# codybloemhard/termdaw

Measured on AMD Instinct MI355X. Metric: offline render Msamples/sec (stereo 48 kHz) + % HBM roofline, 64-vertex graph, higher is better.
Workload: dtype f32; 1 GPU; BASELINE config 2: 64 sampleloop -> 1 normalize, 60 s @48 kHz, bl 1024, 16-bit PCM out; 1 project(s) per GPU per step (project p of the job on rank p mod N, seed offset 64*p); frames_per_project=2880512, projects_per_gpu=1, vertices_per_project=65, normalize=one launch, output=int16 PCM in HBM, parallelism=project p on rank p mod N; one RCCL all-reduce(max) of the 1-entry peak table

## Files before the change

termdaw_amd/csrc/compile.cpp:

```cpp
#include "chorus_math.h"
#include "compile.h"
#include "delay_math.h"
#include "eq_math.h"
#include "sat_math.h"

#include <math.h>
#include <stdlib.h>
#include <string.h>

#include <algorithm>
#include <chrono>
#include <limits>

using namespace tdk;

namespace tde {

const char* const kFamilyName[F_COUNT] = {"k_sample_loop", "k_sample_multi", "k_sample_lerp", "k_debug_sine",
                                           "k_synth",       "k_sampsyn", "k_adsr_env", "k_sine_probe", "k_sum",          "k_scale",       "k_norm_fix",
                                           "k_adsr",        "k_band_pass",    "k_band_spec", "k_band_fix", "k_band_fill", "k_band_scan", "k_quantise", "k_band_audit", "k_stems", "k_sources", "k_loudness",
                                           "k_master_detect", "k_master_scan", "k_master_carry", "k_master_apply",
                                           "k_comp_detect", "k_comp_carry_y1", "k_comp_env", "k_comp_carry_yl", "k_comp_apply",
                                           "k_eq_local", "k_eq_carry", "k_eq_apply",
                                           "k_delay_local", "k_delay_carry", "k_delay_apply",
// ... 1366 lines not shown
            if (!adsr_through.empty()) term_mode[vi] = ins.size() == 1 ? TERMS_ADSR1 : TERMS_WITH_ADSR;
            for (const auto& th : adsr_through) {
                const size_t a = th.second;
                const Vertex& av = g->vertices[a];
                AdsrVDesc x{};
                x.tab.n_int = vt[a].n_int;
                x.k = 1u;
                x.sr = (uint32_t)sr;
                x.bl = (uint32_t)bl;
                x.use_off = av.use_off;
                x.use_max = av.use_max;
                x.wet = av.wet;
                x.conf = av.conf;
                x.pg = make_pg(av.gain, av.angle);
                adsr_fill_run_consts(&x);
                x.env = env_of[a];
                const size_t in_off = st.put(std::vector<InTerm>{plain_term(g->edges[a][0])});
                const size_t o = st.alloc(sizeof x);
                memcpy(&st.b[o], &x, sizeof x);
                ptr_field(o, offsetof(AdsrVDesc, ins), in_off);
                const size_t t = o + offsetof(AdsrVDesc, tab);
                tab_field(t, offsetof(IntervalTab, istart), vt[a], vt[a].istart_off);
                tab_field(t, offsetof(IntervalTab, tile_first), vt[a], vt[a].tile_first_off);
                tab_field(t, offsetof(IntervalTab, ivoff), vt[a], vt[a].ivoff_off);
                tab_field(t, offsetof(IntervalTab, voices), vt[a], vt[a].voices_off);
                ptr_field(ins_off[vi] + th.first * sizeof(InTerm), offsetof(InTerm, len), o);
            }
        }
        for (size_t vi : norm_pending) {
            const Vertex& v = g->vertices[vi];
            uint32_t mode = 1u;
            if (g->spec_normalize && !is_scan) {
                const uint32_t tm = term_mode[vi];
                const bool wide = (tm == TERMS_ALL_LOOP16 || tm == TERMS_ALL_LOOP32) && bl == (size_t)kTileFrames &&
                                  M >= (size_t)1800 * kTileFrames && M < ((size_t)1 << 31);
                if (v.peak_known && !v.has_init_override) mode = 3u;
                else if (!wide && g->single_pass_normalize && bl == (size_t)kTileFrames && M < ((size_t)1 << 31)) {
                    const int tpw = norm1_tiles_per_workgroup(tm, (uint32_t)M);
                    if (tpw) { mode = 5u; norm_tpw[vi] = tpw; }
                } else if (wide && g->single_pass_normalize) {
                    const bool packed = tm == TERMS_ALL_LOOP16;
                    const int nq = (packed && M >= (size_t)2600 * kTileFrames) ? 4 : 2;
                    const size_t gx = (M + (size_t)kTileFrames * nq - 1) / ((size_t)kTileFrames * nq);
                    mode = (size_t)sum16w_resident_capacity(nq, packed) >= gx ? 5u : 4u;
                }
            }
            norm_mode[vi] = mode;
            fam_v[mode == 1u ? F_SCALE : F_NORMFIX].push_back(vi);
        }
        std::map<size_t, std::pair<size_t, size_t>> norm_scratch;
        std::map<size_t, SumDesc> sum_desc_of;
        size_t band_desc_off = 0;
        uint32_t max_nseg = 0;
        for (int fam = 0; fam < F_COUNT; ++fam) {
            auto& vs = fam_v[fam];
            if (fam == F_BAND_FILL) continue;
            if (fam == F_BAND_FIX) vs = fam_v[F_BAND_SPEC];
            if (vs.empty() && !(fam == F_SUM && !fam_v[F_BAND_SPEC].empty())) continue;
            size_t off = 0;
            switch (fam) {
                case F_LOOP: {
                    std::vector<LoopDesc> d;
                    for (size_t vi : vs) {
                        const Vertex& v = g->vertices[vi];
                        const SampleEntry& s = sb->samples[v.sample_index];
                        const bool fits32 = s.len <= 0xFFFFFFFFull && vt[vi].t0 + M + kTileFrames <= 0xFFFFFFFFull;
                        const uint32_t magic = fits32 ? (s.len >= 2 ? (uint32_t)(0x100000000ull / s.len) : 0xFFFFFFFFu) : 0u;
                        d.push_back({s.d, g->vbuf[vi], s.len, vt[vi].t0, magic, {0, 0, 0}, make_pg(v.gain, v.angle)});
                    }
                    off = st.put(d);
                } break;
                case F_MULTI: {
                    std::vector<MultiDesc> d;
                    for (size_t vi : vs) {
                        const Vertex& v = g->vertices[vi];
                        const SampleEntry& s = sb->samples[v.sample_index];
                        d.push_back({s.d, g->vbuf[vi], nullptr, s.len, vt[vi].n_hits, 0, make_pg(v.gain, v.angle), nullptr});
                    }
// ... 858 lines not shown
                        x.voices = (uint32_t)v.chorus_voices;
                        x.shape = (uint32_t)v.chorus_shape;
                        x.wet = v.wet;
                        x.D0 = c[0];
                        x.A = c[1];
                        x.f = c[2];
                        x.stereo = (double)v.chorus_stereo;
                        x.inv_v = 1.0 / (double)v.chorus_voices;
                        x.pg = make_pg(v.gain, v.angle);
                        d.push_back(x);
                    }
                    off = st.put(d);
                    for (size_t i = 0; i < vs.size(); ++i) ptr_field(off + i * sizeof(ChorusDesc), offsetof(ChorusDesc, ins), ins_off[vs[i]]);
                    if (multi) add_launch(F_CHORUS_SUM, off, (int)vs.size(), 0, lv);
                    add_launch(F_CHORUS, off, (int)vs.size(), chorus_aux(n_tiles, !multi), lv);
                    continue;
                }
                default: continue;
            }
            if (fam == F_SUM || fam == F_ADSR) {
                const size_t dsz = fam == F_SUM ? sizeof(SumDesc) : sizeof(AdsrVDesc);
                size_t b = 0;
                while (b < vs.size()) {
                    size_t e2 = b;
                    bool wide_ok = true;
                    auto m4 = [&](size_t vi) { return fam == F_SUM && norm_mode.count(vi) && norm_mode[vi] >= 4u; };
                    auto tpw_of = [&](size_t vi) { return (fam == F_SUM && norm_tpw.count(vi)) ? norm_tpw[vi] : 0; };
                    while (e2 < vs.size() && term_mode[vs[e2]] == term_mode[vs[b]] && m4(vs[e2]) == m4(vs[b]) && tpw_of(vs[e2]) == tpw_of(vs[b])) {
                        wide_ok = wide_ok && (g->vertices[vs[e2]].kind != K_NORMALIZE || bl == (size_t)kTileFrames);
                        wide_ok = wide_ok && !(fam == F_SUM && band_plan.count(vs[e2]));
                        ++e2;
                    }
                    add_launch(fam, off + b * dsz, (int)(e2 - b),
                               term_mode[vs[b]] | (wide_ok ? 0x100u : 0u) | (m4(vs[b]) ? 0x200u : 0u) | ((uint32_t)tpw_of(vs[b]) << 12), lv);
                    b = e2;
                }
                continue;
            }
            add_launch(fam, off, (int)vs.size(), max_nseg, lv);
        }
        for (float2* t : level_tmp) g->free_bufs.push_back(t);
        for (size_t vi : g->order)
            if (g->vbuf[vi] && last_use[vi] == lv && !tapped[vi]) {
                g->free_bufs.push_back(g->vbuf[vi]);
                last_use[vi] = -2;
            }
    }
    for (float2* b : env_bufs) g->free_bufs.push_back(b);
    const Vertex& outv = g->vertices[(size_t)g->output_vertex];
    if (pcm_dst && qmode && outv.kind != K_NORMALIZE) {
        std::vector<QuantDesc> d{{g->vbuf[(size_t)g->output_vertex], pcm_dst, amplitude, (uint32_t)qmode}};
        add_launch(F_QUANT, st.put(d), 1, 0u, g->n_levels);
    }
    const bool stem_pcm = pcm_dst && qmode;
    if (!g->stems.empty() && !is_scan && (stem_pcm || g->stem_f32_wanted)) {
        const size_t qbytes = qmode == 1 ? 4 : 8;
        std::vector<StemDesc> d;
        for (size_t k = 0; k < g->stems.size(); ++k) {
            const size_t sv = g->stems[k];
            StemDesc x{};
            if (inlined[sv] == 1) {
                x.src = loop_term(sv);
            } else {
                if (inlined[sv] || !g->vbuf[sv]) return fail("termdaw_amd: internal: a stem vertex was not materialised");
                x.src.p = g->vbuf[sv];
                x.src.kind = 0u;
            }
// ... 139 lines not shown
```

termdaw_amd/csrc/engine.cpp:

```cpp
#include <chrono>

#include "engine.h"
#include "chorus_math.h"
#include "comm.h"
#include "compile.h"
#include "delay_math.h"
#include "devmem.h"
#include "eq_math.h"
#include "midi.h"
#include "sat_math.h"

#include <math.h>
#include <stdlib.h>
#include <string.h>

#include <algorithm>
#include <map>
#include <tuple>
#include <mutex>
#include <condition_variable>
#include <atomic>
#include <thread>
#include <limits>

// ... 799 lines not shown
                    }
                    in_one_grid |= 1ull << ((size_t)pick[kd] - li);
                }
                const bool z = zero_in_sources && li == 0;
                Prof pr(prof, F_SOURCES, stream);
                if (debug_sync() & 4) fprintf(stderr, "L k_sources M=%u\n", M0);
                launch_sources(P, M0, z ? ar.d + sync_at : nullptr, z ? (cb.sync_bytes + 15) & ~(size_t)15 : 0, stream);
                if (debug_sync() & 4) { (void)hipStreamSynchronize(stream); fprintf(stderr, "ok\n"); }
            }
        }
        for (size_t q = li; q < lj; ++q) {
            const Launch& L = launches[q];
            if (in_one_grid & (1ull << (q - li))) continue;
            if (L.fam == F_NORMFIX && (L.aux & 1u)) {
                ar.pending_fix.push_back({L.off, L.n, L.M, L.bl});
                continue;
            }
            const void* d = ar.d + L.off;
            hipStream_t s = stream;
            Prof pr(prof, L.fam, s);
            if (debug_sync() & 4) fprintf(stderr, "L %s n=%d M=%u bl=%u aux=%x\n", kFamilyName[L.fam], L.n, L.M, L.bl, L.aux);
            struct Crumb { hipStream_t s; ~Crumb() { if (debug_sync() & 4) { (void)hipStreamSynchronize(s); fprintf(stderr, "ok\n"); } } } crumb{s};
            switch (L.fam) {
                case F_LOOP: launch_sample_loop((const LoopDesc*)d, L.n, L.M, s); break;
                case F_MULTI: launch_sample_multi((const MultiDesc*)d, L.n, L.M, s); break;
                case F_LERP: launch_sample_lerp((const LerpDesc*)d, L.n, L.M, s); break;
                case F_SINE: launch_debug_sine((const SineDesc*)d, L.n, L.M, L.bl, s); break;
                case F_SYNTH: launch_synth((const SynthDesc*)d, L.n, L.M, (L.aux & 1u) != 0u, s); break;
                case F_SAMPSYN: launch_sampsyn((const SampsynDesc*)d, L.n, L.M, s); break;
                case F_ENV: launch_adsr_env((const AdsrVDesc*)d, L.n, L.M, s); break;
                case F_PROBE: launch_sine_probe((const ProbeDesc*)d, L.n, L.M, L.aux, s); break;
                case F_SUM:
                    if (L.aux >> 12) launch_norm1((const SumDesc*)d, L.n, L.M, L.aux & 0xFFu, (int)(L.aux >> 12), sum_tag, s);
                    else launch_sum((const SumDesc*)d, L.n, L.M, L.bl, L.aux & 0xFFu, (L.aux & 0x100u) != 0u, (L.aux & 0x200u) != 0u, sum_tag, s);
                    break;
                case F_SCALE: launch_scale((const ScaleDesc*)d, L.n, L.M, L.bl, L.is_scan, s); break;
                case F_NORMFIX: launch_norm_fix((const SumDesc*)d, L.n, L.M, L.bl, s); break;
                case F_ADSR: launch_adsr((const AdsrVDesc*)d, L.n, L.M, L.aux & 0xFFu, s); break;
                case F_BAND: launch_band_pass((const BandDesc*)d, L.n, L.M, s); break;
                case F_BAND_SPEC: launch_band_spec((const BandSpecDesc*)d, L.n, L.M, L.aux, s); break;
                case F_BAND_FIX: launch_band_fix((const BandSpecDesc*)d, L.n, L.M, L.aux, s); break;
                case F_BAND_FILL: break;
                case F_BAND_SCAN:
                    if (L.aux & 0x10000u) launch_band_chain((const BandScanDesc*)d, L.n, L.M, L.aux & 0xFFu, (L.aux & 0x20000u) != 0u, s);
                    else launch_band_scan((const BandScanDesc*)d, L.n, L.M, L.aux & 0xFFu, (int)((L.aux >> 8) & 0xFFu), s);
                    break;
                case F_QUANT: launch_quantise((const QuantDesc*)d, L.n, L.M, s); break;
                case F_AUDIT: launch_band_audit((const AuditHead*)d, L.n, s); break;
                case F_STEMS: launch_stems((const StemDesc*)d, L.n, L.M, s); break;
                case F_COMP_DETECT: launch_comp_detect((const CompDesc*)d, L.n, L.aux, s); break;
                case F_COMP_CARRY1:
                case F_COMP_CARRY2: launch_master_carry((const MasterDesc*)d, L.n, s); break;
                case F_COMP_ENV: launch_comp_env((const CompDesc*)d, L.n, L.aux, s); break;
                case F_COMP_APPLY: launch_comp_apply((const CompDesc*)d, L.n, L.aux, s); break;
                case F_EQ_LOCAL: launch_eq_local((const EqDesc*)d, L.n, L.aux, s); break;
                case F_EQ_CARRY: launch_eq_carry((const EqDesc*)d, L.n, s); break;
                case F_EQ_APPLY: launch_eq_apply((const EqDesc*)d, L.n, L.aux, s); break;
                case F_DELAY_LOCAL: launch_delay_local((const DelayDesc*)d, L.n, L.aux, s); break;
                case F_DELAY_CARRY: launch_delay_carry((const DelayDesc*)d, L.n, L.aux, s); break;
                case F_DELAY_APPLY: launch_delay_apply((const DelayDesc*)d, L.n, L.aux & ~kDelaySingleBit, (L.aux & kDelaySingleBit) != 0u, s); break;
                case F_SAT_SUM: launch_sat_sum((const SatDesc*)d, L.n, L.M, s); break;
                case F_SAT: launch_sat((const SatDesc*)d, L.n, (L.aux >> 24) & 15u, L.aux & 0xFFFFFu, ((L.aux >> 20) & 15u) * 128u, (L.aux & kSatTermsBit) != 0u, s); break;
                case F_SAT1: launch_sat1((const SatDesc*)d, L.n, L.M, s); break;
                case F_CHORUS_SUM: launch_chorus_sum((const ChorusDesc*)d, L.n, L.M, s); break;
                case F_CHORUS: launch_chorus((const ChorusDesc*)d, L.n, L.aux & 0xFFFFFu, L.M, (L.aux & kChorusTermsBit) != 0u, s); break;
            }
        }
// ... 1679 lines not shown
    return ok ? 1 : fail("td_device_sinf: HIP error");
}
void td_trim_memory(void) { tde::mem_trim(); }
size_t td_cached_memory_bytes(void) { return tde::mem_cached_bytes(); }
size_t td_graph_device_bytes(const td_graph* g) { return g->device_bytes + g->arena.device_bytes; }

int td_graph_band_guard_stats(const td_graph* g, double out[4]) {
    out[0] = (double)g->guard.audits;
    out[1] = (double)g->guard.redos;
    out[2] = (double)g->guard.last_est;
    out[3] = (double)g->guard.max_est;
    return 1;
}
int td_graph_band_stats(const td_graph* gc, uint32_t out[3]) {
    td_graph* g = const_cast<td_graph*>(gc);
    out[0] = out[1] = out[2] = 0;
    if (g->band_stats_off.empty() || !g->band_stats_base) return 1;
    if (!ensure_device(g->device)) return 0;
    TD_HIP(hipStreamSynchronize(g->stream));
    for (size_t so : g->band_stats_off) {
        uint32_t s[4];
        TD_HIP(hipMemcpy(s, g->band_stats_base + so, 16, hipMemcpyDeviceToHost));
        for (int i = 0; i < 3; ++i) out[i] += s[i];
    }
    return 1;
}

struct OptionRef { const char* key; int kind; void* p; };
static std::vector<OptionRef> option_table(td_graph* g) {
    return {
        {"fuse_sources", 0, &g->fuse_sources}, {"packed_samples", 0, &g->packed_samples}, {"band_mode", 1, &g->band_mode},
        {"band_guard_ppb", 2, &g->band_guard_ppb}, {"sine_mode", 1, &g->sine_mode}, {"output_f32", 0, &g->output_f32},
        {"max_chunk_frames", 3, &g->max_chunk_frames},
        {"debug.norm", 1, &g->norm_debug}, {"debug.band_scan", 1, &g->band_scan_debug}, {"debug.one_grid_sources", 0, &g->one_grid_sources}, {"debug.inline_probe", 0, &g->inline_probe},
        {"debug.inline_adsr", 0, &g->inline_adsr}, {"debug.spec_normalize", 0, &g->spec_normalize},
        {"debug.single_pass_normalize", 0, &g->single_pass_normalize}, {"debug.fuse_normalize", 0, &g->fuse_normalize},
        {"debug.table_cache", 0, &g->table_cache}, {"debug.band_serial", 0, &g->band_serial}, {"debug.band_chain", 0, &g->band_chain}, {"debug.band_scan_nf", 1, &g->band_scan_nf},
        {"debug.delay_tile", 2, &g->delay_tile}, {"debug.sat_tile", 2, &g->sat_tile}, {"debug.chorus_tile", 2, &g->chorus_tile},
        {"debug.band_quick", 2, &g->band_quick}, {"debug.band_short", 2, &g->band_short}, {"debug.band_medium", 2, &g->band_medium},
        {"debug.band_warmup", 2, &g->band_warmup}, {"debug.band_depth", 2, &g->band_depth},
        {"debug.stem_taps", 2, &g->stem_taps},
    };
}
int td_graph_set_option(td_graph* g, const char* key, long value) {
    const std::string k = key ? key : "";
    if (k == "debug.stem_taps") return fail("td_graph_set_option: debug.stem_taps is read-only");
    if (k == "band_mode") {
        if (value != 0 && value != 1 && value != 2) return fail("band_mode must be 0 (exact), 1 (scan) or 2 (guarded scan)");
        if (g->guard.armed && !drain(g)) return 0;
        g->band_mode = (int)value;
        return 1;
    }
    if (k == "sine_mode") {
        if (value != 0 && value != 1 && value != 2) return fail("td_graph_set_option: sine_mode is 0 (fast), 1 (glibc's sinf) or 2 (fast under the guard)");
        if (g->guard.armed && !drain(g)) return 0;
        g->sine_mode = (int)value;
        for (auto& v : g->vertices)
            if (v.kind == K_DEBUG_SINE || v.kind == K_SYNTH) v.exact_sin = value == 1;
        return 1;
    }
    if (k == "band_guard_ppb") { g->band_guard_ppb = value > 0 ? (unsigned)std::min<long>(value, 1000000000L) : 0u; return 1; }
    if (k == "max_chunk_frames") {
        if (value < 1) return fail("max_chunk_frames must be >= 1");
        g->max_chunk_frames = (size_t)value;
        return 1;
    }
    if (k == "debug.band_scan_nf") {
        if (value != 8 && value != 16) return fail("debug.band_scan_nf must be 8 or 16");
        g->band_scan_nf = (int)value;
        return 1;
    }
    if (k == "debug.delay_tile") {
        if (value != 8 && value != 16 && value != 32 && value != 64) return fail("debug.delay_tile must be 8, 16, 32 or 64");
        g->delay_tile = (unsigned)value;
        return 1;
    }
    if (k == "debug.sat_tile") {
        if (value != 128 && value != 256 && value != 384) return fail("debug.sat_tile must be 128, 256 or 384");
        g->sat_tile = (unsigned)value;
        return 1;
    }
    if (k == "debug.chorus_tile") {
        if (value != 256 && value != 512 && value != 1024) return fail("debug.chorus_tile must be 256, 512 or 1024");
        g->chorus_tile = (unsigned)value;
        return 1;
    }
    if (k == "debug.band_live_exp") { g->band_live_thr = value >= 38 ? 0.0f : powf(10.0f, -(float)value); return 1; }
    if (k == "debug.band_short") { g->band_short = value > 0 ? (unsigned)value : 64u; return 1; }
    if (k == "debug.band_medium") { g->band_medium = value > 0 ? (unsigned)value : 30u; return 1; }
    if (k == "debug.band_depth") { g->band_depth = value > 0 ? (unsigned)value : 100u; return 1; }
    if (k == "debug.band_warmup") { g->band_warmup = value > 0 ? (unsigned)value : 150u; return 1; }
    for (const OptionRef& o : option_table(g)) {
        if (k != o.key) continue;
        switch (o.kind) {
            case 0: *(bool*)o.p = value != 0; break;
            case 1: *(int*)o.p = (int)value; break;
            case 2: *(unsigned*)o.p = value > 0 ? (unsigned)value : 0u; break;
            default: *(size_t*)o.p = value > 0 ? (size_t)value : 0; break;
        }
        return 1;
    }
    return fail("unknown option \"" + k + "\"");
// ... 472 lines not shown
```

termdaw_amd/csrc/engine.h:

```cpp
#pragma once
#include <string.h>

#include <deque>
#include <memory>
#include <utility>
#include <map>
#include <string>
#include <vector>

#include "../../include/termdaw_amd.h"
#include "kernels.h"

namespace tde {

extern thread_local std::string g_error;
int fail(const std::string& msg);

size_t f32_as_usize(float x);

struct SampleEntry {
    float2* d = nullptr;
    size_t len = 0;
    uint32_t* d16 = nullptr;
    float scale_l = 0.0f, scale_r = 0.0f;
// ... 309 lines not shown
    float2* d_resampled = nullptr;
    std::vector<size_t> stems;
    uint8_t* d_stem_pcm = nullptr;
    size_t stem_pcm_cap = 0, stem_stride = 0, stem_pcm_bytes = 0;
    uint32_t* d_stem_peak = nullptr;
    size_t stem_peak_cap = 0;
    float2* d_stem_f32 = nullptr;
    size_t stem_f32_cap = 0, stem_f32_stride = 0;
    bool stem_f32_wanted = false;
    size_t stems_rendered = 0;
    size_t chunk_frame0 = 0;
    unsigned stem_taps = 0;
    size_t loud_frames = 0, loud_sr = 0;
    int loud_bits = 16;
    uint8_t* d_loud = nullptr;
    size_t loud_cap = 0;
    std::vector<std::vector<double>> momentary;
    bool master_kept = false;
    uint8_t* d_master_src = nullptr;
    size_t master_src_cap = 0;
    uint8_t* d_master = nullptr;
    size_t master_cap = 0;
    size_t device_bytes = 0;
    bool fuse_sources = true;
    bool packed_samples = true;
    bool inline_adsr = true;
    bool output_f32 = true;
    bool table_cache = true;
    bool spec_normalize = true;
    bool inline_probe = true;
    bool one_grid_sources = true;
    bool fuse_normalize = true;
    bool single_pass_normalize = true;
    int norm_debug = 0;
    bool defer_fix = true;
    float band_live_thr = 1e-9f;
    unsigned band_depth = 100;
    unsigned band_medium = 30;
    unsigned band_quick = 12;
    unsigned band_short = 40;
    unsigned band_warmup = 150;
    bool band_serial = false;
    int sine_mode = 1;
    int band_mode = 0;
    unsigned band_guard_ppb = 200;
    tde::Guard guard;
    bool band_chain = true;
    int band_scan_nf = 16;
    int band_scan_debug = 0;
    std::vector<size_t> band_stats_off;
    const uint8_t* band_stats_base = nullptr;
    size_t max_chunk_frames = (size_t)1 << 24;
    tde::ProfCtx prof;
    tde::Staging staging;
    std::vector<tde::BlockCursor> cursor;
    std::vector<size_t> cursor_starts;
    double host_ms[4] = {0, 0, 0, 0};
    size_t host_chunks = 0;
    tde::HostSnapshot snapshot;
};

struct td_batch {
    int device = 0;
    hipStream_t stream = nullptr;
    std::vector<td_graph*> graphs;
    std::vector<const td_samplebank*> sbs;
// ... 34 lines not shown
```

termdaw_amd/csrc/kernels.h:

```cpp
#pragma once
#include <hip/hip_runtime.h>
#include <stdint.h>
#include "adsr_math.h"

namespace tdk {

constexpr int kThreads = 256;
constexpr int kTileFrames = 1024;
constexpr uint32_t kBandMaxSegs = 131072;
constexpr uint32_t kBandMaxS = 1024;

struct PanGain {
    float l_amp, r_amp, gain;
    uint32_t flags;
};

struct InTerm {
    const float2* p;
    uint64_t len;
    uint64_t t0;
    PanGain pg;
    uint32_t kind;
    uint32_t magic;
    float scale_l, scale_r;
};
enum TermMode : uint32_t { TERMS_MIXED = 0, TERMS_ALL_EDGE = 1, TERMS_ALL_LOOP32 = 2, TERMS_ALL_LOOP16 = 3,
                           TERMS_EDGE_FEW = 4,
                           TERMS_ADSR1 = 5,
                           TERMS_WITH_ADSR = 6 };

struct NormState { float max, scan_max; uint32_t violated, ticket; };

struct BandRespParam {
    double ql[8], qh[8];
    double gl, gh;
// ... 435 lines not shown
void launch_band_scan(const BandScanDesc* d, int n_desc, uint32_t frames, uint32_t term_mode, int nf, hipStream_t s);
int band_scan_resident_capacity(int nf);
void launch_band_chain(const BandScanDesc* d, int n_desc, uint32_t frames, uint32_t term_mode, bool guarded, hipStream_t s);
inline uint32_t band_scan_tile_frames(int nf) { return (uint32_t)nf * (uint32_t)kThreads; }

constexpr int kSincLen = 256, kSincOver = 256;
struct ResampleDesc {
    const float2* in;
    float2* out;
    const float* table;
    uint64_t len, nout, from, to;
};
void launch_resample(const ResampleDesc& d, hipStream_t s);

enum PcmFormat : uint32_t { PCM_F32 = 0, PCM_U8 = 1, PCM_S16 = 2, PCM_S24 = 3, PCM_S32 = 4 };
void launch_pcm_decode(const uint8_t* raw, float* linear, uint32_t n_values, uint32_t format, hipStream_t s);
void launch_sample_split(const float* linear, uint32_t channels, uint32_t src_l, uint32_t src_r, float* l, float* r,
                         uint32_t nl, uint32_t nr, hipStream_t s);
void launch_absmax(const float* v, uint32_t n, float* out, hipStream_t s);
void launch_abs_sum_serial(const float* v, uint32_t n, float* out, hipStream_t s);
void launch_add_planar(const float* a, const float* b, float* out, uint32_t n, hipStream_t s);
void launch_sample_pack(const float* l, const float* r, const float* max_l, const float* max_r, float2* frames,
                        uint32_t n, hipStream_t s);
void launch_sample_pack16(const float* l, const float* r, uint32_t* packed, uint32_t n, uint32_t* not_int16, hipStream_t s);

void launch_peak_table(const float* const* src, float* table, uint32_t n_total, uint32_t n_own, uint32_t first, uint32_t stride,
                       hipStream_t s);

void launch_band_spec(const BandSpecDesc* d, int n_desc, uint32_t frames, uint32_t max_nseg, hipStream_t s);
void launch_band_fix(const BandSpecDesc* d, int n_desc, uint32_t frames, uint32_t max_nseg, hipStream_t s);
int norm1_tiles_per_workgroup(uint32_t term_mode, uint32_t frames);
void launch_norm1(const SumDesc* d, int n_desc, uint32_t frames, uint32_t term_mode, int tpw, uint32_t tag, hipStream_t s);
int sum16w_resident_capacity(int nq, bool packed);
void launch_sum(const SumDesc* d, int n_desc, uint32_t frames, uint32_t bl, uint32_t term_mode, bool wide_ok, bool must_wide, uint32_t tag, hipStream_t s);
void launch_scale(const ScaleDesc* d, int n_desc, uint32_t frames, uint32_t bl, int is_scan, hipStream_t s);
void launch_norm_fix(const SumDesc* d, int n_desc, uint32_t frames, uint32_t bl, hipStream_t s);
void launch_quantise(const QuantDesc* d, int n_desc, uint32_t frames, hipStream_t s);
__attribute__((weak)) void launch_stems(const StemDesc* d, int n_desc, uint32_t frames, hipStream_t s);
__attribute__((weak)) void launch_loudness(const LoudDesc* d, int n_desc, uint32_t max_tiles, hipStream_t s);
__attribute__((weak)) void launch_master_detect(const MasterDesc* d, int n_desc, uint32_t max_tiles, hipStream_t s);
__attribute__((weak)) void launch_master_scan(const MasterDesc* d, int n_desc, uint32_t max_tiles, hipStream_t s);
__attribute__((weak)) void launch_master_carry(const MasterDesc* d, int n_desc, hipStream_t s);
__attribute__((weak)) void launch_master_apply(const MasterDesc* d, int n_desc, uint32_t max_tiles, hipStream_t s);
__attribute__((weak)) void launch_comp_detect(const CompDesc* d, int n_desc, uint32_t max_tiles, hipStream_t s);
__attribute__((weak)) void launch_comp_env(const CompDesc* d, int n_desc, uint32_t max_tiles, hipStream_t s);
__attribute__((weak)) void launch_comp_apply(const CompDesc* d, int n_desc, uint32_t max_tiles, hipStream_t s);
__attribute__((weak)) void launch_eq_local(const EqDesc* d, int n_desc, uint32_t max_tiles, hipStream_t s);
__attribute__((weak)) void launch_eq_carry(const EqDesc* d, int n_desc, hipStream_t s);
__attribute__((weak)) void launch_eq_apply(const EqDesc* d, int n_desc, uint32_t max_tiles, hipStream_t s);
constexpr uint32_t kDelaySingleBit = 0x80000000u;
__attribute__((weak)) void launch_delay_local(const DelayDesc* d, int n_desc, uint32_t max_groups, hipStream_t s);
__attribute__((weak)) void launch_delay_carry(const DelayDesc* d, int n_desc, uint32_t max_groups, hipStream_t s);
__attribute__((weak)) void launch_delay_apply(const DelayDesc* d, int n_desc, uint32_t max_groups, bool single, hipStream_t s);
constexpr uint32_t kSatTermsBit = 0x80000000u;
constexpr uint32_t kSatInlineFrames = 4096;
inline uint32_t sat_aux(uint32_t n_tiles, uint32_t F, uint32_t R, bool terms) {
    return n_tiles | ((F / 128u) << 20) | (R << 24) | (terms ? kSatTermsBit : 0u);
}
__attribute__((weak)) void launch_sat_sum(const SatDesc* d, int n_desc, uint32_t frames, hipStream_t s);
__attribute__((weak)) void launch_sat(const SatDesc* d, int n_desc, uint32_t R, uint32_t n_tiles, uint32_t F, bool terms, hipStream_t s);
__attribute__((weak)) void launch_sat1(const SatDesc* d, int n_desc, uint32_t frames, hipStream_t s);
constexpr uint32_t kChorusTermsBit = 0x80000000u;
inline uint32_t chorus_aux(uint32_t n_tiles, bool terms) { return n_tiles | (terms ? kChorusTermsBit : 0u); }
__attribute__((weak)) void launch_chorus_sum(const ChorusDesc* d, int n_desc, uint32_t frames, hipStream_t s);
__attribute__((weak)) void launch_chorus(const ChorusDesc* d, int n_desc, uint32_t n_tiles, uint32_t frames, bool terms, hipStream_t s);
void launch_sinf(const float* in, float* out, uint32_t n, int exact, hipStream_t s);
// ... 25 lines not shown
```

termdaw_amd/csrc/kernels.hip:

```cpp
#include "kernels.h"

#include <algorithm>

namespace tdk {

#define TD_DEV __device__ __forceinline__

TD_DEV float2 epilogue(float2 v, const PanGain& pg) {
    if (pg.flags & 1u) { v.x *= pg.l_amp; v.y *= pg.r_amp; }
    if (pg.flags & 2u) { v.x *= pg.gain;  v.y *= pg.gain;  }
    return v;
}
TD_DEV float4 epilogue4(float4 v, const PanGain& pg) {
    float2 a = epilogue(make_float2(v.x, v.y), pg), b = epilogue(make_float2(v.z, v.w), pg);
    return make_float4(a.x, a.y, b.x, b.y);
}

#define TD_GLOBAL __attribute__((address_space(1)))
typedef float f4v __attribute__((ext_vector_type(4)));
typedef float f2v __attribute__((ext_vector_type(2)));
typedef unsigned int u2v __attribute__((ext_vector_type(2)));
typedef int i4v __attribute__((ext_vector_type(4)));
typedef int i2v __attribute__((ext_vector_type(2)));
TD_DEV float4 gload4(const void* p) { const f4v v = *reinterpret_cast<const f4v TD_GLOBAL*>((const TD_GLOBAL char*)p); return make_float4(v.x, v.y, v.z, v.w); }
// ... 304 lines not shown
#pragma unroll
        for (int f = 0; f < 4; ++f) {
            f2v v = cvt16(w[f]) * sc;
            v = v * am;
            v = v * gn;
            c[f] = c[f] + v;
        }
    };
    auto gather = [&](uint32_t j, uint32_t w[4]) {
        const uint32_t len = (uint32_t)ins[j].len;
        loop16_quad(reinterpret_cast<const uint32_t*>(ins[j].p), len, barrett_mod((uint32_t)ins[j].t0 + m, len, ins[j].magic), w);
    };
    uint32_t j = 0;
    for (; j + 4 <= k; j += 4) {
        uint32_t w[4][4];
#pragma unroll
        for (int u = 0; u < 4; ++u) gather(j + u, w[u]);
#pragma unroll
        for (int u = 0; u < 4; ++u) add_term(j + u, w[u]);
    }
    for (; j < k; ++j) {
        uint32_t w[4];
        gather(j, w);
        add_term(j, w);
    }
    acc0 = zero_tail(make_float4(c[0].x, c[0].y, c[1].x, c[1].y), m, M);
    acc1 = zero_tail(make_float4(c[2].x, c[2].y, c[3].x, c[3].y), m + 2u, M);
}

TD_DEV uint32_t step256(uint32_t len, uint32_t magic) {
    const uint32_t r = 256u - __umulhi(256u, magic) * len;
    return r >= len ? r - len : r;
}
template <int NQ>
TD_DEV uint32_t quad_frame(uint32_t m, int q) { return NQ == 4 ? m + 256u * (uint32_t)q : m + 4u * (uint32_t)q; }
template <int NQ>
TD_DEV uint32_t pair_frame(uint32_t m, int p) { return quad_frame<NQ>(m, p >> 1) + 2u * (uint32_t)(p & 1); }
template <int NQ>
TD_DEV void sum_terms16w(TermTab ins, uint32_t k, uint32_t m, uint32_t M, float4 acc[2 * NQ]) {
    f2v c[4 * NQ];
#pragma unroll
    for (int f = 0; f < 4 * NQ; ++f) { c[f].x = 0.f; c[f].y = 0.f; }
    auto add_term = [&](uint32_t j, const uint32_t w[4 * NQ]) {
        f2v sc, am, gn;
        sc.x = ins[j].scale_l; sc.y = ins[j].scale_r;
        am.x = ins[j].pg.l_amp; am.y = ins[j].pg.r_amp;
        gn.x = gn.y = ins[j].pg.gain;
#pragma unroll
        for (int f = 0; f < 4 * NQ; ++f) {
            f2v v = cvt16(w[f]) * sc;
            v = v * am;
            v = v * gn;
            c[f] = c[f] + v;
        }
    };
    auto gather = [&](uint32_t j, uint32_t w[4 * NQ]) {
        const uint32_t len = (uint32_t)ins[j].len;
        const uint32_t idx = barrett_mod((uint32_t)ins[j].t0 + m, len, ins[j].magic);
        if (NQ == 4) {
            const uint32_t* p = reinterpret_cast<const uint32_t*>(ins[j].p);
            const uint32_t step = step256(len, ins[j].magic);
            uint32_t i = idx;
#pragma unroll
            for (int q = 0; q < NQ; ++q) {
                loop16_quad(p, len, i, w + 4 * q);
                i += step;
                i = min(i, i - len);
            }
            return;
        }
#pragma unroll
        for (int q = 0; q < NQ; ++q) loop16_quad(reinterpret_cast<const uint32_t*>(ins[j].p), len, idx + 4u * q, w + 4 * q);
    };
    uint32_t j = 0;
    constexpr int B = 4;
    for (; j + B <= k; j += B) {
        uint32_t w[B][4 * NQ];
#pragma unroll
        for (int u = 0; u < B; ++u) gather(j + u, w[u]);
#pragma unroll
        for (int u = 0; u < B; ++u) add_term(j + u, w[u]);
    }
    for (; j < k; ++j) { uint32_t w[4 * NQ]; gather(j, w); add_term(j, w); }
#pragma unroll
    for (int q = 0; q < 2 * NQ; ++q) acc[q] = zero_tail(make_float4(c[2 * q].x, c[2 * q].y, c[2 * q + 1].x, c[2 * q + 1].y), pair_frame<NQ>(m, q), M);
}

template <int NQ>
TD_DEV void sum_terms32w(TermTab ins, uint32_t k, uint32_t m, uint32_t M, float4 acc[2 * NQ]) {
    f4v c[2 * NQ];
#pragma unroll
    for (int q = 0; q < 2 * NQ; ++q) { c[q].x = 0.f; c[q].y = 0.f; c[q].z = 0.f; c[q].w = 0.f; }
    constexpr int B = NQ >= 4 ? 1 : 2;
    auto gather = [&](uint32_t j, f4v x[2 * NQ]) {
        const uint32_t len = (uint32_t)ins[j].len;
        const uint32_t idx = barrett_mod((uint32_t)ins[j].t0 + m, len, ins[j].magic);
        const float2* p = ins[j].p + idx;
#pragma unroll
        for (int q = 0; q < 2 * NQ; ++q) {
            const float4 v = gload4u(p + 2 * q);
            x[q].x = v.x; x[q].y = v.y; x[q].z = v.z; x[q].w = v.w;
        }
    };
    auto add_term = [&](uint32_t j, const f4v x[2 * NQ]) {
        f4v am, gn;
        am.x = am.z = ins[j].pg.l_amp; am.y = am.w = ins[j].pg.r_amp;
        gn.x = gn.y = gn.z = gn.w = ins[j].pg.gain;
#pragma unroll
        for (int q = 0; q < 2 * NQ; ++q) {
            f4v v = x[q] * am;
            v = v * gn;
            c[q] = c[q] + v;
        }
    };
    uint32_t j = 0;
    for (; j + B <= k; j += B) {
        f4v x[B][2 * NQ];
#pragma unroll
// ... 152 lines not shown
    if (tiles_per_block) {
        float pk = 0.0f;
        if (m0 < M) pk = absmax4(pk, a0);
        if (m1 < M) pk = absmax4(pk, a1);
        pk = wave_max(pk);
        __shared__ float wmax[kThreads / 64];
        if ((threadIdx.x & 63) == 0) wmax[threadIdx.x >> 6] = pk;
        __syncthreads();
        if (threadIdx.x == 0) {
            pk = fmaxf(fmaxf(wmax[0], wmax[1]), fmaxf(wmax[2], wmax[3]));
            uint32_t b = blockIdx.x / tiles_per_block;
            if (tiles_per_block == 1) d.peaks[b] = pk;
            else atomicMax(reinterpret_cast<unsigned int*>(d.peaks + b), __float_as_uint(pk));
            if (spec && pk > spec_init) const_cast<NormState*>(d.state)->violated = 1u;
        }
    } else {
        if (spec) {
            const float pk = fmaxf(m0 < M ? absmax4(0.0f, a0) : 0.0f, m1 < M ? absmax4(0.0f, a1) : 0.0f);
            if (pk > spec_init) const_cast<NormState*>(d.state)->violated = 1u;
        }
        const float v[8] = {a0.x, a0.y, a0.z, a0.w, a1.x, a1.y, a1.z, a1.w};
#pragma unroll
        for (int f = 0; f < 4; ++f) {
            uint32_t m = (f < 2 ? m0 : m1) + (f & 1);
            if (m < M) {
                float pk = fmaxf(fmaxf(0.0f, fabsf(v[2 * f])), fabsf(v[2 * f + 1]));
                atomicMax(reinterpret_cast<unsigned int*>(d.peaks + m / bl), __float_as_uint(pk));
            }
        }
    }
}

template <int NQ, bool PACKED = true>
__global__ __launch_bounds__(kThreads) void k_sum16w(const SumDesc* __restrict__ descs, uint32_t M, uint32_t tag) {
    const SumDesc& d = descs[blockIdx.y];
    constexpr int SH = (NQ == 4 && PACKED) ? 4 : 1;
    const uint32_t m = SH == 4 ? blockIdx.x * (kTileFrames * NQ) + (threadIdx.x >> 6) * kTileFrames + 4u * (threadIdx.x & 63u)
                               : blockIdx.x * (kTileFrames * NQ) + 4u * NQ * threadIdx.x;
    const float spec_init_early = d.mode >= 4 ? (d.use_init ? d.init_max : gload1(&d.state->max)) : 0.0f;
    float4 a[2 * NQ];
    if (PACKED) sum_terms16w<NQ>(term_tab(d.ins), d.k, m, M, a);
    else sum_terms32w<NQ>(term_tab(d.ins), d.k, m, M, a);
    if (d.mode == 0) {
#pragma unroll
        for (int q = 0; q < 2 * NQ; ++q) store_pair(d.out, pair_frame<SH>(m, q), M, epilogue4(a[q], d.pg));
        return;
    }
    float pk = 0.0f;
#pragma unroll
    for (int q = 0; q < 2 * NQ; ++q) if (pair_frame<SH>(m, q) < M) pk = absmax4(pk, a[q]);
    float spec_init = 0.0f;
    if (d.mode >= 4) {
        const float init = spec_init_early;
        __shared__ float wm4[kThreads / 64], pm4[kThreads / 64];
        __shared__ uint32_t bad4;
        const uint32_t wave = threadIdx.x >> 6;
        const float pw = wave_max(pk);
        if ((threadIdx.x & 63) == 0) wm4[wave] = pw;
        if (threadIdx.x == 0) bad4 = 0u;
        __syncthreads();
        constexpr uint32_t wpb = 4 / NQ;
        float pb[NQ], T = 0.0f;
#pragma unroll
        for (int b = 0; b < NQ; ++b) {
            float p = wm4[b * wpb];
            for (uint32_t u = 1; u < wpb; ++u) p = fmaxf(p, wm4[b * wpb + u]);
            pb[b] = p;
            T = fmaxf(T, p);
        }
        if (threadIdx.x < (uint32_t)NQ) {
// ... 4332 lines not shown
    for (int tpw : {1, 2, 4})
        if ((uint32_t)norm1_capacity(term_mode, tpw) >= (nt + (uint32_t)tpw - 1u) / (uint32_t)tpw) return tpw;
    return 0;
}
template <int TMODE, int TPW>
static void launch_norm1_of(const SumDesc* d, int n, uint32_t frames, uint32_t tag, hipStream_t s) {
    static const auto kern = &k_norm1<TMODE, TPW>;
    const uint32_t nt = (frames + kTileFrames - 1) / kTileFrames, gx = (nt + TPW - 1) / TPW;
    const int per = std::max(1, norm1_capacity_of<TMODE, TPW>() / (int)gx);
    for (int o = 0; o < n; o += per)
        hipLaunchKernelGGL(kern, dim3(gx, std::min(per, n - o)), dim3(kThreads), 0, s, d + o, frames, nt, tag);
}
template <int TMODE>
static void launch_norm1_mode(const SumDesc* d, int n, uint32_t frames, int tpw, uint32_t tag, hipStream_t s) {
    if (tpw == 1) launch_norm1_of<TMODE, 1>(d, n, frames, tag, s);
    else if (tpw == 2) launch_norm1_of<TMODE, 2>(d, n, frames, tag, s);
    else launch_norm1_of<TMODE, 4>(d, n, frames, tag, s);
}
void launch_norm1(const SumDesc* d, int n, uint32_t frames, uint32_t term_mode, int tpw, uint32_t tag, hipStream_t s) {
    if (!n || !frames) return;
    switch (term_mode) {
        case TERMS_ALL_EDGE: launch_norm1_mode<TERMS_ALL_EDGE>(d, n, frames, tpw, tag, s); break;
        case TERMS_ALL_LOOP32: launch_norm1_mode<TERMS_ALL_LOOP32>(d, n, frames, tpw, tag, s); break;
        case TERMS_ALL_LOOP16: launch_norm1_mode<TERMS_ALL_LOOP16>(d, n, frames, tpw, tag, s); break;
        case TERMS_EDGE_FEW: launch_norm1_mode<TERMS_EDGE_FEW>(d, n, frames, tpw, tag, s); break;
        case TERMS_ADSR1: launch_norm1_mode<TERMS_ADSR1>(d, n, frames, tpw, tag, s); break;
        case TERMS_WITH_ADSR: launch_norm1_mode<TERMS_WITH_ADSR>(d, n, frames, tpw, tag, s); break;
        default: launch_norm1_mode<TERMS_MIXED>(d, n, frames, tpw, tag, s); break;
    }
}
void launch_sum(const SumDesc* d, int n, uint32_t frames, uint32_t bl, uint32_t term_mode, bool wide_ok, bool must_wide, uint32_t tag, hipStream_t s) {
    if (!n || !frames) return;
    const uint32_t tpb = (bl % kTileFrames == 0) ? bl / kTileFrames : 0;
    static const int env_nq = getenv("TD_FORCE_NQ") ? atoi(getenv("TD_FORCE_NQ")) : 0;
    const int forced_nq = (must_wide && env_nq == 1) ? 0 : env_nq;
    if (must_wide) wide_ok = true;
    static const int slice_env = getenv("TD_SUM_SLICE") ? atoi(getenv("TD_SUM_SLICE")) : 0;
    switch (term_mode) {
        case TERMS_ALL_EDGE: TD_BATCHED(HIP_KERNEL_NAME(k_sum<TERMS_ALL_EDGE>), tiles(frames), kThreads, d, n, frames, bl, tpb); break;
        case TERMS_ALL_LOOP32:
            if (wide_ok && frames >= 1800u * kTileFrames) {
                const uint32_t gx = (frames + kTileFrames * 2 - 1) / (kTileFrames * 2);
                const int per = must_wide ? std::max(1, sum16w_resident_capacity(2, false) / (int)gx) : n;
                for (int o = 0; o < n; o += per)
                    hipLaunchKernelGGL(k_sum32w_2, dim3(gx, std::min(per, n - o)), dim3(kThreads), 0, s, d + o, frames, tag);
            }
            else
                TD_BATCHED(HIP_KERNEL_NAME(k_sum<TERMS_ALL_LOOP32>), tiles(frames), kThreads, d, n, frames, bl, tpb);
            break;
        case TERMS_ALL_LOOP16:
            if (wide_ok && (forced_nq ? forced_nq == 4 : frames >= 2600u * kTileFrames)) {
                const uint32_t gx = (frames + kTileFrames * 4 - 1) / (kTileFrames * 4);
                int per = slice_env > 0 ? slice_env : (int)std::max(1u, (256u * 4u) / gx);
                if (must_wide) per = std::max(1, std::min(per, sum16w_resident_capacity(4, true) / (int)gx));
                for (int o = 0; o < n; o += per)
                    hipLaunchKernelGGL(HIP_KERNEL_NAME(k_sum16w<4>), dim3(gx, std::min(per, n - o)), dim3(kThreads), 0, s, d + o, frames, tag);
            } else if (wide_ok && (forced_nq ? forced_nq == 2 : frames >= 1800u * kTileFrames)) {
                const uint32_t gx = (frames + kTileFrames * 2 - 1) / (kTileFrames * 2);
                int per = slice_env > 0 ? slice_env : (int)std::max(1u, (256u * 4u) / gx);
                if (must_wide) per = std::max(1, std::min(per, sum16w_resident_capacity(2, true) / (int)gx));
                for (int o = 0; o < n; o += per)
                    hipLaunchKernelGGL(HIP_KERNEL_NAME(k_sum16w<2>), dim3(gx, std::min(per, n - o)), dim3(kThreads), 0, s, d + o, frames, tag);
            }
            else
                TD_BATCHED(HIP_KERNEL_NAME(k_sum<TERMS_ALL_LOOP16>), tiles(frames), kThreads, d, n, frames, bl, tpb);
            break;
        case TERMS_EDGE_FEW: TD_BATCHED(HIP_KERNEL_NAME(k_sum<TERMS_EDGE_FEW>), tiles(frames), kThreads, d, n, frames, bl, tpb); break;
        case TERMS_ADSR1: TD_BATCHED(HIP_KERNEL_NAME(k_sum<TERMS_ADSR1>), tiles(frames), kThreads, d, n, frames, bl, tpb); break;
        case TERMS_WITH_ADSR: TD_BATCHED(HIP_KERNEL_NAME(k_sum<TERMS_WITH_ADSR>), tiles(frames), kThreads, d, n, frames, bl, tpb); break;
        default: TD_BATCHED(HIP_KERNEL_NAME(k_sum<TERMS_MIXED>), tiles(frames), kThreads, d, n, frames, bl, tpb); break;
    }
}
void launch_scale(const ScaleDesc* d, int n, uint32_t frames, uint32_t bl, int is_scan, hipStream_t s) {
    if (!n || !frames) return;
    TD_BATCHED(k_scale, tiles(frames), kThreads, d, n, frames, bl, frames / bl, is_scan);
}
void launch_norm_fix(const SumDesc* d, int n, uint32_t frames, uint32_t bl, hipStream_t s) {
    if (!n || !frames) return;
    TD_BATCHED(k_norm_fix, std::min(tiles(frames), 512u), kThreads, d, n, frames, bl, frames / bl);
}
__global__ __launch_bounds__(kThreads) void k_debug_verify(const uint32_t* __restrict__ p, uint32_t n_words, const uint32_t* __restrict__ seg_sums,
                                                           uint32_t* __restrict__ report) {
    __shared__ uint32_t bad_seg;
    if (threadIdx.x == 0) bad_seg = 0xFFFFFFFFu;
    __syncthreads();
    const uint32_t n_seg = (n_words + 63u) / 64u;
    const uint32_t wave = threadIdx.x / 64u, lane = threadIdx.x % 64u;
    for (uint32_t sg = wave; sg < n_seg; sg += kThreads / 64u) {
        const uint32_t i = sg * 64u + lane;
        uint32_t v = i < n_words ? p[i] * (2u * lane + 1u) : 0u;
#pragma unroll
        for (int off = 32; off > 0; off >>= 1) v += __shfl_xor(v, off, 64);
        if (lane == 0u && v != seg_sums[sg]) atomicMin(&bad_seg, sg);
    }
    __syncthreads();
// ... 335 lines not shown
```

Baseline: 49390 Msamples/s.

## Unify wide-sum form selection and use strided quad layout for NQ=2 packed sums

Moves the wide-sum choice (quads per lane, resident normalize mode, slice size) into one shared helper used by both the compiler and the launcher, and adds a debug option that forces 2 or 4 quads. The packed k_sum16w<2> kernel now uses the same 256-frame strided quad layout and step-based gather as the NQ=4 path, with a configurable batch depth and an occupancy hint in launch_bounds. The intent is coalesced per-quad loads and more resident waves for the two-quad variant. The trade-off is that the occupancy hint may cap registers and cause spills, and the different frame mapping could change memory access patterns.

Result: no change. 49420 Msamples/s (median of 2 runs) (+0.1%).

```diff
diff --git a/termdaw_amd/csrc/compile.cpp b/termdaw_amd/csrc/compile.cpp
--- a/termdaw_amd/csrc/compile.cpp
+++ b/termdaw_amd/csrc/compile.cpp
@@ -1422,18 +1422,16 @@
             uint32_t mode = 1u;
             if (g->spec_normalize && !is_scan) {
                 const uint32_t tm = term_mode[vi];
-                const bool wide = (tm == TERMS_ALL_LOOP16 || tm == TERMS_ALL_LOOP32) && bl == (size_t)kTileFrames &&
-                                  M >= (size_t)1800 * kTileFrames && M < ((size_t)1 << 31);
+                const bool packed = tm == TERMS_ALL_LOOP16;
+                const SumWideForm form = ((packed || tm == TERMS_ALL_LOOP32) && bl == (size_t)kTileFrames && M < ((size_t)1 << 31))
+                                             ? sum_wide_form(M, packed, sum16w_resident_capacity(2, packed), packed ? sum16w_resident_capacity(4, true) : 0, g->sum_wide)
+                                             : SumWideForm{0, 4u, 1};
+                const bool wide = form.nq != 0;
                 if (v.peak_known && !v.has_init_override) mode = 3u;
                 else if (!wide && g->single_pass_normalize && bl == (size_t)kTileFrames && M < ((size_t)1 << 31)) {
                     const int tpw = norm1_tiles_per_workgroup(tm, (uint32_t)M);
                     if (tpw) { mode = 5u; norm_tpw[vi] = tpw; }
-                } else if (wide && g->single_pass_normalize) {
-                    const bool packed = tm == TERMS_ALL_LOOP16;
-                    const int nq = (packed && M >= (size_t)2600 * kTileFrames) ? 4 : 2;
-                    const size_t gx = (M + (size_t)kTileFrames * nq - 1) / ((size_t)kTileFrames * nq);
-                    mode = (size_t)sum16w_resident_capacity(nq, packed) >= gx ? 5u : 4u;
-                }
+                } else if (wide && g->single_pass_normalize) mode = form.mode;
             }
             norm_mode[vi] = mode;
             fam_v[mode == 1u ? F_SCALE : F_NORMFIX].push_back(vi);
@@ -2358,7 +2356,8 @@
                         ++e2;
                     }
                     add_launch(fam, off + b * dsz, (int)(e2 - b),
-                               term_mode[vs[b]] | (wide_ok ? 0x100u : 0u) | (m4(vs[b]) ? 0x200u : 0u) | ((uint32_t)tpw_of(vs[b]) << 12), lv);
+                               term_mode[vs[b]] | (wide_ok ? 0x100u : 0u) | (m4(vs[b]) ? 0x200u : 0u) | (fam == F_SUM && g->sum_wide == 2 ? 0x400u : 0u) |
+                                   (fam == F_SUM && g->sum_wide == 4 ? 0x800u : 0u) | ((uint32_t)tpw_of(vs[b]) << 12), lv);
                     b = e2;
                 }
                 continue;
diff --git a/termdaw_amd/csrc/engine.cpp b/termdaw_amd/csrc/engine.cpp
--- a/termdaw_amd/csrc/engine.cpp
+++ b/termdaw_amd/csrc/engine.cpp
@@ -855,7 +855,8 @@
                 case F_PROBE: launch_sine_probe((const ProbeDesc*)d, L.n, L.M, L.aux, s); break;
                 case F_SUM:
                     if (L.aux >> 12) launch_norm1((const SumDesc*)d, L.n, L.M, L.aux & 0xFFu, (int)(L.aux >> 12), sum_tag, s);
-                    else launch_sum((const SumDesc*)d, L.n, L.M, L.bl, L.aux & 0xFFu, (L.aux & 0x100u) != 0u, (L.aux & 0x200u) != 0u, sum_tag, s);
+                    else launch_sum((const SumDesc*)d, L.n, L.M, L.bl, (L.aux & 0xFFu) | ((L.aux & 0x400u) ? 2u << 8 : (L.aux & 0x800u) ? 4u << 8 : 0u),
+                                    (L.aux & 0x100u) != 0u, (L.aux & 0x200u) != 0u, sum_tag, s);
                     break;
                 case F_SCALE: launch_scale((const ScaleDesc*)d, L.n, L.M, L.bl, L.is_scan, s); break;
                 case F_NORMFIX: launch_norm_fix((const SumDesc*)d, L.n, L.M, L.bl, s); break;
@@ -2601,7 +2602,7 @@
         {"fuse_sources", 0, &g->fuse_sources}, {"packed_samples", 0, &g->packed_samples}, {"band_mode", 1, &g->band_mode},
         {"band_guard_ppb", 2, &g->band_guard_ppb}, {"sine_mode", 1, &g->sine_mode}, {"output_f32", 0, &g->output_f32},
         {"max_chunk_frames", 3, &g->max_chunk_frames},
-        {"debug.norm", 1, &g->norm_debug}, {"debug.band_scan", 1, &g->band_scan_debug}, {"debug.one_grid_sources", 0, &g->one_grid_sources}, {"debug.inline_probe", 0, &g->inline_probe},
+        {"debug.norm", 1, &g->norm_debug}, {"debug.sum_wide", 1, &g->sum_wide}, {"debug.band_scan", 1, &g->band_scan_debug}, {"debug.one_grid_sources", 0, &g->one_grid_sources}, {"debug.inline_probe", 0, &g->inline_probe},
         {"debug.inline_adsr", 0, &g->inline_adsr}, {"debug.spec_normalize", 0, &g->spec_normalize},
         {"debug.single_pass_normalize", 0, &g->single_pass_normalize}, {"debug.fuse_normalize", 0, &g->fuse_normalize},
         {"debug.table_cache", 0, &g->table_cache}, {"debug.band_serial", 0, &g->band_serial}, {"debug.band_chain", 0, &g->band_chain}, {"debug.band_scan_nf", 1, &g->band_scan_nf},
@@ -2637,6 +2638,11 @@
     if (k == "debug.band_scan_nf") {
         if (value != 8 && value != 16) return fail("debug.band_scan_nf must be 8 or 16");
         g->band_scan_nf = (int)value;
+        return 1;
+    }
+    if (k == "debug.sum_wide") {
+        if (value != 0 && value != 2 && value != 4) return fail("debug.sum_wide must be 0 (by length), 2 or 4 (quads per lane)");
+        g->sum_wide = (int)value;
         return 1;
     }
     if (k == "debug.delay_tile") {
diff --git a/termdaw_amd/csrc/engine.h b/termdaw_amd/csrc/engine.h
--- a/termdaw_amd/csrc/engine.h
+++ b/termdaw_amd/csrc/engine.h
@@ -365,6 +365,7 @@
     bool one_grid_sources = true;
     bool fuse_normalize = true;
     bool single_pass_normalize = true;
+    int sum_wide = 0;
     int norm_debug = 0;
     bool defer_fix = true;
     float band_live_thr = 1e-9f;
diff --git a/termdaw_amd/csrc/kernels.h b/termdaw_amd/csrc/kernels.h
--- a/termdaw_amd/csrc/kernels.h
+++ b/termdaw_amd/csrc/kernels.h
@@ -1,6 +1,8 @@
 #pragma once
 #include <hip/hip_runtime.h>
 #include <stdint.h>
+
+#include <algorithm>
 #include "adsr_math.h"
 
 namespace tdk {
@@ -502,6 +504,21 @@
 int norm1_tiles_per_workgroup(uint32_t term_mode, uint32_t frames);
 void launch_norm1(const SumDesc* d, int n_desc, uint32_t frames, uint32_t term_mode, int tpw, uint32_t tag, hipStream_t s);
 int sum16w_resident_capacity(int nq, bool packed);
+constexpr uint32_t kSumWide2FromTiles = 1800, kSumWide4FromTiles = 2600;
+struct SumWideForm { int nq; uint32_t mode; int per; };
+inline SumWideForm sum_wide_form(uint64_t frames, bool packed, int cap2, int cap4, int forced) {
+    const uint64_t nt = (frames + kTileFrames - 1) / kTileFrames;
+    int nq = 0;
+    if (forced == 2 || forced == 4) nq = packed ? forced : 2;
+    else if (packed && nt >= kSumWide4FromTiles) nq = 4;
+    else if (nt >= kSumWide2FromTiles) nq = 2;
+    if (!nq) return {0, 4u, 1};
+    const uint64_t gx = (nt + (uint64_t)nq - 1) / (uint64_t)nq;
+    const uint64_t cap = (uint64_t)std::max(nq == 4 ? cap4 : cap2, 0);
+    const bool resident = gx <= cap;
+    const uint64_t slice = packed ? (1024u / gx > 0 ? 1024u / gx : 1u) : (resident ? cap / gx : 1u);
+    return {nq, resident ? 5u : 4u, (int)(resident && cap / gx < slice ? cap / gx : slice)};
+}
 void launch_sum(const SumDesc* d, int n_desc, uint32_t frames, uint32_t bl, uint32_t term_mode, bool wide_ok, bool must_wide, uint32_t tag, hipStream_t s);
 void launch_scale(const ScaleDesc* d, int n_desc, uint32_t frames, uint32_t bl, int is_scan, hipStream_t s);
 void launch_norm_fix(const SumDesc* d, int n_desc, uint32_t frames, uint32_t bl, hipStream_t s);
diff --git a/termdaw_amd/csrc/kernels.hip b/termdaw_amd/csrc/kernels.hip
--- a/termdaw_amd/csrc/kernels.hip
+++ b/termdaw_amd/csrc/kernels.hip
@@ -360,12 +360,19 @@
     const uint32_t r = 256u - __umulhi(256u, magic) * len;
     return r >= len ? r - len : r;
 }
-template <int NQ>
-TD_DEV uint32_t quad_frame(uint32_t m, int q) { return NQ == 4 ? m + 256u * (uint32_t)q : m + 4u * (uint32_t)q; }
-template <int NQ>
-TD_DEV uint32_t pair_frame(uint32_t m, int p) { return quad_frame<NQ>(m, p >> 1) + 2u * (uint32_t)(p & 1); }
+template <int SH>
+TD_DEV uint32_t quad_frame(uint32_t m, int q) { return SH == 4 ? m + 256u * (uint32_t)q : m + 4u * (uint32_t)q; }
+template <int SH>
+TD_DEV uint32_t pair_frame(uint32_t m, int p) { return quad_frame<SH>(m, p >> 1) + 2u * (uint32_t)(p & 1); }
+#ifndef TD_SUM2_B
+#define TD_SUM2_B 4
+#endif
+#ifndef TD_SUM2_WAVES
+#define TD_SUM2_WAVES 6
+#endif
 template <int NQ>
 TD_DEV void sum_terms16w(TermTab ins, uint32_t k, uint32_t m, uint32_t M, float4 acc[2 * NQ]) {
+    constexpr int SH = 4;
     f2v c[4 * NQ];
 #pragma unroll
     for (int f = 0; f < 4 * NQ; ++f) { c[f].x = 0.f; c[f].y = 0.f; }
@@ -385,23 +392,20 @@
     auto gather = [&](uint32_t j, uint32_t w[4 * NQ]) {
         const uint32_t len = (uint32_t)ins[j].len;
         const uint32_t idx = barrett_mod((uint32_t)ins[j].t0 + m, len, ins[j].magic);
-        if (NQ == 4) {
-            const uint32_t* p = reinterpret_cast<const uint32_t*>(ins[j].p);
-            const uint32_t step = step256(len, ins[j].magic);
-            uint32_t i = idx;
-#pragma unroll
-            for (int q = 0; q < NQ; ++q) {
-                loop16_quad(p, len, i, w + 4 * q);
+        const uint32_t* p = reinterpret_cast<const uint32_t*>(ins[j].p);
+        const uint32_t step = step256(len, ins[j].magic);
+        uint32_t i = idx;
+#pragma unroll
+        for (int q = 0; q < NQ; ++q) {
+            loop16_quad(p, len, i, w + 4 * q);
+            if (q + 1 < NQ) {
                 i += step;
                 i = min(i, i - len);
             }
-            return;
-        }
-#pragma unroll
-        for (int q = 0; q < NQ; ++q) loop16_quad(reinterpret_cast<const uint32_t*>(ins[j].p), len, idx + 4u * q, w + 4 * q);
+        }
     };
     uint32_t j = 0;
-    constexpr int B = 4;
+    constexpr int B = NQ == 4 ? 4 : TD_SUM2_B;
     for (; j + B <= k; j += B) {
         uint32_t w[B][4 * NQ];
 #pragma unroll
@@ -411,7 +415,7 @@
     }
     for (; j < k; ++j) { uint32_t w[4 * NQ]; gather(j, w); add_term(j, w); }
 #pragma unroll
-    for (int q = 0; q < 2 * NQ; ++q) acc[q] = zero_tail(make_float4(c[2 * q].x, c[2 * q].y, c[2 * q + 1].x, c[2 * q + 1].y), pair_frame<NQ>(m, q), M);
+    for (int q = 0; q < 2 * NQ; ++q) acc[q] = zero_tail(make_float4(c[2 * q].x, c[2 * q].y, c[2 * q + 1].x, c[2 * q + 1].y), pair_frame<SH>(m, q), M);
 }
 
 template <int NQ>
@@ -630,10 +634,10 @@
 }
 
 template <int NQ, bool PACKED = true>
-__global__ __launch_bounds__(kThreads) void k_sum16w(const SumDesc* __restrict__ descs, uint32_t M, uint32_t tag) {
+__global__ __launch_bounds__(kThreads, (NQ == 2 && PACKED) ? TD_SUM2_WAVES : 1) void k_sum16w(const SumDesc* __restrict__ descs, uint32_t M, uint32_t tag) {
     const SumDesc& d = descs[blockIdx.y];
-    constexpr int SH = (NQ == 4 && PACKED) ? 4 : 1;
-    const uint32_t m = SH == 4 ? blockIdx.x * (kTileFrames * NQ) + (threadIdx.x >> 6) * kTileFrames + 4u * (threadIdx.x & 63u)
+    constexpr int SH = PACKED ? 4 : 1;
+    const uint32_t m = SH == 4 ? blockIdx.x * (kTileFrames * NQ) + (threadIdx.x >> 6) * (256u * NQ) + 4u * (threadIdx.x & 63u)
                                : blockIdx.x * (kTileFrames * NQ) + 4u * NQ * threadIdx.x;
     const float spec_init_early = d.mode >= 4 ? (d.use_init ? d.init_max : gload1(&d.state->max)) : 0.0f;
     float4 a[2 * NQ];
@@ -5032,16 +5036,15 @@
 void launch_sum(const SumDesc* d, int n, uint32_t frames, uint32_t bl, uint32_t term_mode, bool wide_ok, bool must_wide, uint32_t tag, hipStream_t s) {
     if (!n || !frames) return;
     const uint32_t tpb = (bl % kTileFrames == 0) ? bl / kTileFrames : 0;
-    static const int env_nq = getenv("TD_FORCE_NQ") ? atoi(getenv("TD_FORCE_NQ")) : 0;
-    const int forced_nq = (must_wide && env_nq == 1) ? 0 : env_nq;
+    const int forced = (int)((term_mode >> 8) & 7u);
+    term_mode &= 0xFFu;
     if (must_wide) wide_ok = true;
-    static const int slice_env = getenv("TD_SUM_SLICE") ? atoi(getenv("TD_SUM_SLICE")) : 0;
     switch (term_mode) {
         case TERMS_ALL_EDGE: TD_BATCHED(HIP_KERNEL_NAME(k_sum<TERMS_ALL_EDGE>), tiles(frames), kThreads, d, n, frames, bl, tpb); break;
         case TERMS_ALL_LOOP32:
-            if (wide_ok && frames >= 1800u * kTileFrames) {
+            if (const SumWideForm f = sum_wide_form(frames, false, wide_ok ? sum16w_resident_capacity(2, false) : 0, 0, wide_ok ? forced : 0); wide_ok && f.nq) {
                 const uint32_t gx = (frames + kTileFrames * 2 - 1) / (kTileFrames * 2);
-                const int per = must_wide ? std::max(1, sum16w_resident_capacity(2, false) / (int)gx) : n;
+                const int per = must_wide ? f.per : n;
                 for (int o = 0; o < n; o += per)
                     hipLaunchKernelGGL(k_sum32w_2, dim3(gx, std::min(per, n - o)), dim3(kThreads), 0, s, d + o, frames, tag);
             }
@@ -5049,18 +5052,14 @@
                 TD_BATCHED(HIP_KERNEL_NAME(k_sum<TERMS_ALL_LOOP32>), tiles(frames), kThreads, d, n, frames, bl, tpb);
             break;
         case TERMS_ALL_LOOP16:
-            if (wide_ok && (forced_nq ? forced_nq == 4 : frames >= 2600u * kTileFrames)) {
-                const uint32_t gx = (frames + kTileFrames * 4 - 1) / (kTileFrames * 4);
-                int per = slice_env > 0 ? slice_env : (int)std::max(1u, (256u * 4u) / gx);
-                if (must_wide) per = std::max(1, std::min(per, sum16w_resident_capacity(4, true) / (int)gx));
-                for (int o = 0; o < n; o += per)
-                    hipLaunchKernelGGL(HIP_KERNEL_NAME(k_sum16w<4>), dim3(gx, std::min(per, n - o)), dim3(kThreads), 0, s, d + o, frames, tag);
-            } else if (wide_ok && (forced_nq ? forced_nq == 2 : frames >= 1800u * kTileFrames)) {
-                const uint32_t gx = (frames + kTileFrames * 2 - 1) / (kTileFrames * 2);
-                int per = slice_env > 0 ? slice_env : (int)std::max(1u, (256u * 4u) / gx);
-                if (must_wide) per = std::max(1, std::min(per, sum16w_resident_capacity(2, true) / (int)gx));
-                for (int o = 0; o < n; o += per)
-                    hipLaunchKernelGGL(HIP_KERNEL_NAME(k_sum16w<2>), dim3(gx, std::min(per, n - o)), dim3(kThreads), 0, s, d + o, frames, tag);
+            if (const SumWideForm f = wide_ok ? sum_wide_form(frames, true, sum16w_resident_capacity(2, true), sum16w_resident_capacity(4, true), forced)
+                                              : SumWideForm{0, 4u, 1}; f.nq) {
+                const uint32_t gx = (frames + kTileFrames * (uint32_t)f.nq - 1) / (kTileFrames * (uint32_t)f.nq);
+                const int per = f.per;
+                for (int o = 0; o < n; o += per) {
+                    if (f.nq == 4) hipLaunchKernelGGL(HIP_KERNEL_NAME(k_sum16w<4>), dim3(gx, std::min(per, n - o)), dim3(kThreads), 0, s, d + o, frames, tag);
+                    else hipLaunchKernelGGL(HIP_KERNEL_NAME(k_sum16w<2>), dim3(gx, std::min(per, n - o)), dim3(kThreads), 0, s, d + o, frames, tag);
+                }
             }
             else
                 TD_BATCHED(HIP_KERNEL_NAME(k_sum<TERMS_ALL_LOOP16>), tiles(frames), kThreads, d, n, frames, bl, tpb);
```
